# KhutornoyYaroslav/vcm-ts

Measured on AMD Instinct MI355X. Metric: encoded frames/sec at 1920x1080 GOP-32, higher is better.
Workload: dtype f32 (fp16x3 split-MFMA, fp32 accumulate)

## Files before the change

include/dcvc_hip.h:

```cpp
#ifndef DCVC_HIP_H
#define DCVC_HIP_H

#include <stdint.h>

#ifdef __cplusplus
extern "C" {
#endif

#define DCVC_OK 0
#define DCVC_E_ARG (-1)
#define DCVC_E_LAUNCH (-2)
#define DCVC_E_RANGE (-3)

#define DCVC_STATUS_ACT_SATURATED 1

#define DCVC_MAX_SEG 3

#define DCVC_PREC_FP32 0
#define DCVC_PREC_FP16X3 1

typedef struct {
    const float *ptr;
    int32_t C;
    int32_t cs;
} dcvc_seg;

typedef struct {
    dcvc_seg seg[DCVC_MAX_SEG];
    int32_t nseg;
    int32_t N, Hin, Win;
    int32_t in_act;
    float in_slope;
    const float *wpack;
    const float *bpack;
    int32_t ks;
    int32_t stride;
    int32_t Cout;
    int32_t Cout_pad;
    float *out;
    int32_t out_cs;
    int32_t out_act;
    float out_slope;
    int32_t pixel_shuffle;
    const float *res;
    int32_t res_cs;
    const float *res_gate;
    const float *res2;
    int32_t res2_cs;
    int32_t precision;
    int32_t *status;
    float *chan_partial;
    int32_t tile_row0;
    int32_t tile_rows;
    int32_t pair_taps;
} dcvc_conv_args;

int32_t dcvc_conv_tile_rows(int32_t ks, int32_t stride);

int32_t dcvc_conv_chan_partial_parts(int32_t ks, int32_t stride, int32_t Hout, int32_t Wout);
int dcvc_channel_mean_finish(const float *chan_partial, int32_t parts, int32_t row_stride, float *mean, int32_t N,
                             int32_t C, int32_t HW, void *stream);

int64_t dcvc_conv_pack_size(int32_t Cout, int32_t ks, int32_t nseg, const int32_t *seg_C, int32_t *cout_pad);

int dcvc_conv_pack_weights(const float *w, const float *b, int32_t Cout, int32_t ks, int32_t nseg,
                           const int32_t *seg_C, int32_t pixel_shuffle, int32_t precision, float *wpack,
                           float *bpack);

int64_t dcvc_conv_pack_size_paired(int32_t Cout, int32_t Cin, int32_t *cout_pad);
int dcvc_conv_pack_weights_paired(const float *w, const float *b, int32_t Cout, int32_t Cin, float *wpack, float *bpack);

int dcvc_conv2d(const dcvc_conv_args *a, void *stream);
int dcvc_conv_set_lookahead(int32_t mode);

int64_t dcvc_conv_small_pack_bytes(int32_t Cout, int32_t ks, int32_t nseg, const int32_t *seg_C);
int dcvc_conv_small_pack_weights(const float *w, const float *b, int32_t Cout, int32_t ks, int32_t nseg,
                                 const int32_t *seg_C, void *wpack, float *bpack);
int dcvc_conv2d_small(const dcvc_conv_args *a, void *stream);

int64_t dcvc_conv_k32_pack_bytes(int32_t Cout, int32_t ks, int32_t nseg, const int32_t *seg_C, int32_t *cout_pad);
int dcvc_conv_k32_pack_weights(const float *w, const float *b, int32_t Cout, int32_t ks, int32_t nseg,
                               const int32_t *seg_C, int32_t pixel_shuffle, void *wpack, float *bpack);
int dcvc_conv2d_k32(const dcvc_conv_args *a, void *stream);
int dcvc_conv_k32_set_waves(int32_t waves);

int dcvc_warp(const float *src, int32_t src_cs, const float *flow, int32_t flow_cs, float *out, int32_t out_cs,
              int32_t N, int32_t H, int32_t W, int32_t C, void *stream);
int dcvc_up2(const float *src, int32_t src_cs, float *out, int32_t out_cs, float *out2, int32_t out2_cs,
             int32_t N, int32_t H, int32_t W, int32_t C, float scale, void *stream);
int dcvc_down2(const float *src, int32_t src_cs, float *out, int32_t out_cs, int32_t N, int32_t H, int32_t W,
               int32_t C, float scale, int32_t avgpool_order, void *stream);
int dcvc_maxpool2(const float *src, int32_t src_cs, float *out, int32_t out_cs, int32_t N, int32_t H, int32_t W,
                  int32_t C, void *stream);
int dcvc_copy_channels(const float *src, int32_t src_cs, float *out, int32_t out_cs, int64_t npix, int32_t C,
                       void *stream);
int dcvc_nchw_to_nhwc(const float *src, float *out, int32_t out_cs, int32_t N, int32_t C, int32_t H, int32_t W,
                      void *stream);
int dcvc_nhwc_to_nchw(const float *src, int32_t src_cs, float *out, int32_t N, int32_t C, int32_t H, int32_t W,
                      int32_t clamp01, void *stream);

int dcvc_channel_mean(const float *src, int32_t src_cs, float *mean, float *scratch, int32_t N, int32_t HW,
                      int32_t C, void *stream);
int dcvc_se_gate(const float *mean, const float *w1, const float *w2, float *gate, int32_t N, int32_t C,
                 int32_t Cr, void *stream);

int dcvc_scale_channels(const float *src, int32_t src_cs, float *out, int32_t out_cs, const float *q_basic,
                        const float *q_scale, int32_t mode, int32_t N, int32_t HW, int32_t C, void *stream);
int dcvc_scale_channels_map(const float *src, int32_t src_cs, float *out, int32_t out_cs, const float *q_basic,
                            const float *q_scale, int32_t mode, int32_t N, int32_t HW, int32_t C, const float *q_map,
                            int32_t H, int32_t W, void *stream);
int dcvc_round_symbols(const float *z, int32_t z_cs, float *z_hat, int32_t zh_cs, int32_t *sym, int32_t N,
                       int32_t H, int32_t W, int32_t C, void *stream);
int dcvc_symbols_to_nhwc(const int32_t *sym, float *out, int32_t out_cs, int32_t N, int32_t H, int32_t W,
                         int32_t C, void *stream);

typedef struct {
    const float *y;
    int32_t y_cs;
    const float *fusion;
    int32_t fusion_cs;
    const float *spatial;
    int32_t spatial_cs;
    float *params;
    int32_t params_cs;
    float *y_hat;
    float *y_q;
    float *y_res;
    float *scales_hat;
    int32_t *sym;
    int32_t *idx;
    float *out;
    int32_t out_cs;
    const float *q_basic;
    const float *q_scale;
    int32_t N, H, W, C;
    int32_t step;
    const float *idx_edges;
    const float *forced_q;
    const float *q_map;
} dcvc_dual_prior_args;

int dcvc_scale_indexes(const float *scales, int32_t *idx, int64_t n, const float *idx_edges, void *stream);

int dcvc_dual_prior_enc(const dcvc_dual_prior_args *a, void *stream);
int dcvc_dual_prior_dec_index(const dcvc_dual_prior_args *a, void *stream);
int dcvc_dual_prior_dec_apply(const dcvc_dual_prior_args *a, void *stream);

int dcvc_scale_bits(const float *y_q, const float *scales_hat, float *out, float *scratch, int32_t kind, int32_t N,
                    int64_t per_sample, void *stream);
int dcvc_factorized_bits(const float *z_hat, int32_t z_cs, const float *params, float *out, float *scratch, int32_t N,
                         int32_t HW, int32_t C, void *stream);
int dcvc_sq_err(const float *a, int32_t a_cs, const float *b, int32_t b_cs, float *out, float *scratch, int32_t N,
                int32_t HW, int32_t C, void *stream);

int32_t dcvc_cdf_table_cols(void);
int dcvc_build_scale_cdfs(const float *scales, int32_t n_scales, int32_t kind, int32_t *cdf, int32_t *sizes,
                          int32_t *offsets, void *stream);
int dcvc_build_factorized_cdfs(const float *params, int32_t C, int32_t *cdf, int32_t *sizes, int32_t *offsets, void *stream);

const char *dcvc_hip_version(void);

#ifdef __cplusplus
}
#endif
#endif
```

vcm_ts_amd/csrc/conv_small.hip:

```cpp
#include <hip/hip_runtime.h>
#include <stdint.h>
#include <string.h>

#include "dcvc_hip.h"
#include "kernel_common.h"

namespace {

constexpr int KC = 16;

struct SmallK {
    const float *seg_ptr[DCVC_MAX_SEG];
    int seg_C[DCVC_MAX_SEG];
    int seg_cs[DCVC_MAX_SEG];
    int nseg;
    int H, W;
    int in_act;
    float in_slope;
    const char *wpack;
    const float *bpack;
    int Cout;
    float *out;
    int out_cs, out_act;
    float out_slope;
    const float *res;
    int res_cs;
    int *status;
};

template <int KS>
__global__ __launch_bounds__(256, 3) void conv_small(const SmallK a) {
    constexpr int RPW = 2, BH = 4 * RPW, BW = 32, PAD = KS / 2, PH = BH + KS - 1, PW = BW + KS - 1, T = KS * KS;
    constexpr int TPS = KS, NST = KS;
    constexpr int PATCH_F = PH * PW * 16;
    constexpr int SLAB_F = TPS * 4 * 16 * 4;
    __shared__ __attribute__((aligned(16))) float lds[PATCH_F + SLAB_F];
    char *patch = (char *)lds;
    float *wl = lds + PATCH_F;

    const int tid = threadIdx.x, lane = tid & 63, wave = tid >> 6;
    const int x0 = blockIdx.x * BW, y0 = blockIdx.y * BH, img = blockIdx.z;
    const int pr = lane & 15, g = lane >> 4;

    f32x4 acc[RPW][2];
#pragma unroll
    for (int m = 0; m < RPW; ++m)
#pragma unroll
        for (int hf = 0; hf < 2; ++hf) acc[m][hf] = (f32x4){0.f, 0.f, 0.f, 0.f};

    constexpr int NP = (PH * PW * 4 + 255) / 256, NW = (SLAB_F / 4 + 255) / 256;
    f32x4 rp[NP], rw[NW];
    struct Cursor {
        int s, c0, cg, st;
    };
    auto advance = [&](Cursor &k) {
        if (++k.st == NST) {
            k.st = 0;
            ++k.cg;
            k.c0 += KC;
            if (k.c0 >= a.seg_C[k.s]) {
                ++k.s;
                k.c0 = 0;
            }
        }
    };
    int poff[NP];
    unsigned inpic = 0;
#pragma unroll
    for (int u = 0; u < NP; ++u) {
        const int i = tid + u * 256;
        const int p = i >> 2;
        const int py = p / PW, px = p - py * PW;
        const int gy = y0 - PAD + py, gx = x0 - PAD + px;
        const bool ok = i < PH * PW * 4 && gy >= 0 && gy < a.H && gx >= 0 && gx < a.W;
        poff[u] = ok ? gy * a.W + gx : 0;
        inpic |= (ok ? 1u : 0u) << u;
    }
    auto load_patch = [&](const Cursor &k) {
        const int C = a.seg_C[k.s], cs = a.seg_cs[k.s];
        const float *sp = a.seg_ptr[k.s] + (size_t)img * a.H * a.W * cs;
        const int c = k.c0 + (tid & 3) * 4;
        const int cc = c < C ? c : 0;
#pragma unroll
        for (int u = 0; u < NP; ++u) rp[u] = *(const f32x4 *)(sp + (size_t)poff[u] * cs + cc);
    };
    auto store_patch = [&](const Cursor &k) {
        const int C = a.seg_C[k.s];
#pragma unroll
        for (int u = 0; u < NP; ++u) {
            const int i = tid + u * 256;
            if (i < PH * PW * 4) {
                const int qd = i & 3, p = i >> 2;
                const int c = k.c0 + qd * 4;
                f32x4 v = ((inpic >> u) & 1u) && c < C ? rp[u] : (f32x4){0.f, 0.f, 0.f, 0.f};
                if (c + 3 >= C) {
                    if (c + 1 >= C) v[1] = 0.f;
                    if (c + 2 >= C) v[2] = 0.f;
                    v[3] = 0.f;
                }
                if (a.in_act) {
#pragma unroll
                    for (int e = 0; e < 4; ++e) v[e] = act(v[e], a.in_slope);
                }
                f32x4 sv = v * ACT_SCALE;
#pragma unroll
                for (int e = 0; e < 4; ++e) sv[e] = __builtin_amdgcn_fmed3f(sv[e], -F16_MAX, F16_MAX);
                const f16x4 hi = __builtin_convertvector(sv, f16x4);
                const f16x4 lo = __builtin_convertvector(sv - __builtin_convertvector(hi, f32x4), f16x4);
                const int sw = (p >> 1) & 3, h = qd >> 1;
                char *rec = patch + p * 64 + (qd & 1) * 8;
                *(f16x4 *)(rec + ((h ^ sw) << 4)) = hi;
                *(f16x4 *)(rec + (((2 + h) ^ sw) << 4)) = lo;
            }
        }
    };
    auto load_w = [&](const Cursor &k) {
        const f32x4 *wsrc = (const f32x4 *)(a.wpack + ((size_t)(k.cg * T + k.st * TPS)) * 1024);
#pragma unroll
        for (int u = 0; u < NW; ++u) {
            const int i = tid + u * 256;
            if (i < SLAB_F / 4) rw[u] = wsrc[i];
        }
    };
    auto store_w = [&]() {
#pragma unroll
        for (int u = 0; u < NW; ++u) {
            const int i = tid + u * 256;
            if (i < SLAB_F / 4) *(f32x4 *)&wl[i * 4] = rw[u];
        }
    };

    Cursor cur = {0, 0, 0, 0};
    load_patch(cur);
    load_w(cur);
    const f16x8 zero8 = {0, 0, 0, 0, 0, 0, 0, 0};
    while (cur.s < a.nseg) {
        __syncthreads();
        if (cur.st == 0) store_patch(cur);
        store_w();
        __syncthreads();
        Cursor nxt = cur;
        advance(nxt);
        if (nxt.s < a.nseg) {
            if (nxt.st == 0) load_patch(nxt);
            load_w(nxt);
        }
#pragma unroll
        for (int tt = 0; tt < TPS; ++tt) {
            const f16x8 b1 = *(const f16x8 *)&wl[((tt * 4 + (g & 1)) * 16 + pr) * 4];
            const f16x8 b2 = g < 2 ? *(const f16x8 *)&wl[((tt * 4 + 2 + g) * 16 + pr) * 4] : zero8;
#pragma unroll
            for (int m = 0; m < RPW; ++m)
#pragma unroll
                for (int hf = 0; hf < 2; ++hf) {
                    const int p = (wave * RPW + m + cur.st) * PW + hf * 16 + pr + tt;
                    const f16x8 av = *(const f16x8 *)(patch + p * 64 + ((g ^ ((p >> 1) & 3)) << 4));
                    acc[m][hf] = __builtin_amdgcn_mfma_f32_16x16x32_f16(av, b1, acc[m][hf], 0, 0, 0);
                    acc[m][hf] = __builtin_amdgcn_mfma_f32_16x16x32_f16(av, b2, acc[m][hf], 0, 0, 0);
                }
        }
        cur = nxt;
    }

    const float inv_scale = 1.f / (ACT_SCALE * WGT_SCALE);
    const int ch = pr;
    bool sat = false;
    if (ch < a.Cout) {
        const float bias = a.bpack[ch];
#pragma unroll
        for (int m = 0; m < RPW; ++m) {
            const int oy = y0 + wave * RPW + m;
            if (oy >= a.H) continue;
            float rv[2][4];
#pragma unroll
            for (int hf = 0; hf < 2; ++hf)
#pragma unroll
                for (int j = 0; j < 4; ++j) {
                    const int ox = x0 + hf * 16 + g * 4 + j;
                    rv[hf][j] = (a.res && ox < a.W) ? a.res[((size_t)(img * a.H + oy) * a.W + ox) * a.res_cs + ch] : 0.f;
                }
#pragma unroll
            for (int hf = 0; hf < 2; ++hf)
#pragma unroll
                for (int j = 0; j < 4; ++j) {
                    const int ox = x0 + hf * 16 + g * 4 + j;
                    if (ox >= a.W) continue;
                    float v = acc[m][hf][j] * inv_scale + bias;
                    if (a.out_act == 1) v = act(v, a.out_slope);
                    else if (a.out_act == 2) v = fminf(fmaxf(v, 0.f), 1.f);
                    if (a.res) v += rv[hf][j];
                    if (a.status && !(fabsf(v) <= ACT_LIMIT)) sat = true;
                    a.out[((size_t)(img * a.H + oy) * a.W + ox) * a.out_cs + ch] = v;
                }
        }
    }
    if (sat) atomicOr(a.status, DCVC_STATUS_ACT_SATURATED);
}

}

extern "C" int64_t dcvc_conv_small_pack_bytes(int32_t Cout, int32_t ks, int32_t nseg, const int32_t *seg_C) {
    if (Cout <= 0 || Cout > 16 || nseg <= 0 || nseg > DCVC_MAX_SEG || (ks != 3 && ks != 7)) return DCVC_E_ARG;
    int chunks = 0;
    for (int s = 0; s < nseg; ++s) {
        if (seg_C[s] <= 0) return DCVC_E_ARG;
        chunks += (seg_C[s] + KC - 1) / KC;
    }
    return (int64_t)chunks * ks * ks * 1024;
}

extern "C" int dcvc_conv_small_pack_weights(const float *w, const float *b, int32_t Cout, int32_t ks, int32_t nseg,
                                            const int32_t *seg_C, void *wpack, float *bpack) {
    const int64_t total = dcvc_conv_small_pack_bytes(Cout, ks, nseg, seg_C);
    if (total < 0 || !w || !wpack || !bpack) return DCVC_E_ARG;
    const int T = ks * ks;
    int Cin = 0;
    for (int s = 0; s < nseg; ++s) Cin += seg_C[s];
    memset(wpack, 0, (size_t)total);
    for (int n = 0; n < 16; ++n) bpack[n] = (b && n < Cout) ? b[n] : 0.f;
    _Float16 *base = (_Float16 *)wpack;
    int status = DCVC_OK, cg = 0, cin0 = 0;
    for (int s = 0; s < nseg; ++s) {
        for (int c0 = 0; c0 < seg_C[s]; c0 += KC, ++cg)
            for (int t = 0; t < T; ++t)
                for (int cc = 0; cc < KC && c0 + cc < seg_C[s]; ++cc)
                    for (int n = 0; n < Cout; ++n) {
                        float sv = w[((size_t)n * Cin + cin0 + c0 + cc) * T + t] * WGT_SCALE;
                        if (!(fabsf(sv) <= F16_MAX)) { status = DCVC_E_RANGE; sv = sv > 0.f ? F16_MAX : -F16_MAX; }
                        const SplitF16 p = split_f16(sv);
                        const size_t blk = ((size_t)cg * T + t) * 4;
                        base[((blk + (cc >> 3)) * 16 + n) * 8 + (cc & 7)] = p.hi;
                        base[((blk + 2 + (cc >> 3)) * 16 + n) * 8 + (cc & 7)] = p.lo;
                    }
        cin0 += seg_C[s];
    }
    return status;
}

extern "C" int dcvc_conv2d_small(const dcvc_conv_args *a, void *stream) {
    if (!conv_args_ok(a)) return DCVC_E_ARG;
    if (a->out_act < 0 || a->out_act > 2) return DCVC_E_ARG;
    if (a->tile_rows > 0) return DCVC_E_ARG;
    if (a->Cout <= 0 || a->Cout > 16 || (a->ks != 3 && a->ks != 7) || a->stride != 1 || a->pixel_shuffle || a->res_gate ||
        a->res2 || a->chan_partial || a->precision != DCVC_PREC_FP16X3 || a->N <= 0)
        return DCVC_E_ARG;
    SmallK k;
    memset(&k, 0, sizeof(k));
    copy_conv_args(k, a);
    k.H = a->Hin, k.W = a->Win;
    dim3 grid((unsigned)((a->Win + 31) / 32), (unsigned)((a->Hin + 7) / 8), (unsigned)a->N);
    if (a->ks == 7)
        hipLaunchKernelGGL(conv_small<7>, grid, dim3(256), 0, (hipStream_t)stream, k);
    else
        hipLaunchKernelGGL(conv_small<3>, grid, dim3(256), 0, (hipStream_t)stream, k);
    RET_LAUNCH();
}
```

vcm_ts_amd/lib.py:

```python
from __future__ import annotations

import ctypes as C
import functools
import os

HERE = os.path.dirname(os.path.abspath(__file__))
CSRC = os.path.join(HERE, "csrc")


class LibraryMissing(RuntimeError):
    pass


class KernelError(RuntimeError):
    pass


def _load(name):
    path = os.environ.get("DCVC_HIP_LIB") if name == "libdcvc_hip.so" and os.environ.get("DCVC_HIP_LIB") else \
        os.path.join(CSRC, name)
    if not os.path.exists(path):
        raise LibraryMissing(f"{path} not built; run `make -C {CSRC}` (no CPU fallback exists)")
    return C.CDLL(path)


@functools.lru_cache(maxsize=None)
def rans():
    L = _load("libdcvc_rans.so")
    L.dcvc_rans_encoder_create.restype = C.c_void_p
    L.dcvc_rans_encoder_destroy.argtypes = [C.c_void_p]
    L.dcvc_rans_encoder_reset.argtypes = [C.c_void_p]
    L.dcvc_rans_encoder_encode_with_indexes.argtypes = [C.c_void_p, C.c_void_p, C.c_void_p, C.c_int64, C.c_void_p,
                                                        C.c_int32, C.c_int32, C.c_void_p, C.c_void_p]
    L.dcvc_rans_encoder_flush_bound.argtypes = [C.c_void_p]
    L.dcvc_rans_encoder_flush_bound.restype = C.c_int64
    L.dcvc_rans_encoder_flush.argtypes = [C.c_void_p, C.c_void_p, C.c_int64]
    L.dcvc_rans_encoder_flush.restype = C.c_int64
    L.dcvc_rans_decoder_create.restype = C.c_void_p
    L.dcvc_rans_decoder_destroy.argtypes = [C.c_void_p]
    L.dcvc_rans_decoder_set_stream.argtypes = [C.c_void_p, C.c_char_p, C.c_int64]
    L.dcvc_rans_decoder_decode_stream.argtypes = [C.c_void_p, C.c_void_p, C.c_int64, C.c_void_p, C.c_int32,
                                                  C.c_int32, C.c_void_p, C.c_void_p, C.c_void_p]
    L.dcvc_pmf_to_quantized_cdf.argtypes = [C.c_void_p, C.c_int32, C.c_int32, C.c_void_p]
    return L


class Seg(C.Structure):
    _fields_ = [("ptr", C.c_void_p), ("C", C.c_int32), ("cs", C.c_int32)]


class ConvArgs(C.Structure):
    _fields_ = [
        ("seg", Seg * 3), ("nseg", C.c_int32), ("N", C.c_int32), ("Hin", C.c_int32), ("Win", C.c_int32),
        ("in_act", C.c_int32), ("in_slope", C.c_float), ("wpack", C.c_void_p), ("bpack", C.c_void_p),
        ("ks", C.c_int32), ("stride", C.c_int32), ("Cout", C.c_int32), ("Cout_pad", C.c_int32),
        ("out", C.c_void_p), ("out_cs", C.c_int32), ("out_act", C.c_int32), ("out_slope", C.c_float),
        ("pixel_shuffle", C.c_int32), ("res", C.c_void_p), ("res_cs", C.c_int32), ("res_gate", C.c_void_p),
        ("res2", C.c_void_p), ("res2_cs", C.c_int32), ("precision", C.c_int32), ("status", C.c_void_p),
        ("chan_partial", C.c_void_p), ("tile_row0", C.c_int32), ("tile_rows", C.c_int32), ("pair_taps", C.c_int32),
    ]


class DualPriorArgs(C.Structure):
    _fields_ = [
        ("y", C.c_void_p), ("y_cs", C.c_int32), ("fusion", C.c_void_p), ("fusion_cs", C.c_int32),
        ("spatial", C.c_void_p), ("spatial_cs", C.c_int32), ("params", C.c_void_p), ("params_cs", C.c_int32),
        ("y_hat", C.c_void_p), ("y_q", C.c_void_p), ("y_res", C.c_void_p), ("scales_hat", C.c_void_p),
        ("sym", C.c_void_p), ("idx", C.c_void_p), ("out", C.c_void_p), ("out_cs", C.c_int32),
        ("q_basic", C.c_void_p), ("q_scale", C.c_void_p), ("N", C.c_int32), ("H", C.c_int32), ("W", C.c_int32),
        ("C", C.c_int32), ("step", C.c_int32), ("idx_edges", C.c_void_p), ("forced_q", C.c_void_p),
        ("q_map", C.c_void_p),
    ]


class ConvBwdArgs(C.Structure):
    _fields_ = [
        ("dout", C.c_void_p), ("dout_cs", C.c_int32), ("out", C.c_void_p), ("out_cs", C.c_int32),
        ("res", C.c_void_p), ("res_cs", C.c_int32), ("gate", C.c_void_p), ("res2", C.c_void_p), ("res2_cs", C.c_int32),
        ("dres", C.c_void_p), ("dres_cs", C.c_int32), ("dres2", C.c_void_p), ("dres2_cs", C.c_int32),
        ("dpre", C.c_void_p), ("dpre_cs", C.c_int32), ("zs", C.c_int32), ("Hd", C.c_int32), ("Wd", C.c_int32),
        ("N", C.c_int32), ("Ho", C.c_int32), ("Wo", C.c_int32), ("Cout", C.c_int32), ("pixel_shuffle", C.c_int32),
        ("act", C.c_int32), ("slope", C.c_float),
    ]


class WgradArgs(C.Structure):
    _fields_ = [
        ("x", C.c_void_p), ("x_cs", C.c_int32), ("C", C.c_int32), ("in_act", C.c_int32), ("in_slope", C.c_float),
        ("dpre", C.c_void_p), ("dpre_cs", C.c_int32), ("zs", C.c_int32), ("Hd", C.c_int32), ("Wd", C.c_int32),
        ("N", C.c_int32), ("Hin", C.c_int32), ("Win", C.c_int32), ("Ho", C.c_int32), ("Wo", C.c_int32),
        ("Cout", C.c_int32), ("ks", C.c_int32), ("stride", C.c_int32), ("dw", C.c_void_p), ("Cin_total", C.c_int32),
        ("cin_offset", C.c_int32), ("scratch", C.c_void_p), ("scratch_floats", C.c_int64), ("overwrite", C.c_int32),
        ("db", C.c_void_p), ("precision", C.c_int32),
    ]


class PackJob(C.Structure):
    _fields_ = [
        ("w", C.c_void_p), ("b", C.c_void_p), ("Cout", C.c_int32), ("Cin_total", C.c_int32), ("ks", C.c_int32),
        ("nseg", C.c_int32), ("seg_C", C.c_int32 * 3), ("cin_offset", C.c_int32), ("pixel_shuffle", C.c_int32),
        ("precision", C.c_int32), ("transposed", C.c_int32), ("wpack", C.c_void_p), ("bpack", C.c_void_p),
    ]


class DualPriorBwdArgs(C.Structure):
    _fields_ = [
        ("y", C.c_void_p), ("y_cs", C.c_int32), ("fusion", C.c_void_p), ("fusion_cs", C.c_int32),
        ("y_hat", C.c_void_p), ("dout", C.c_void_p), ("dout_cs", C.c_int32), ("dy_res", C.c_void_p),
        ("dscales_hat", C.c_void_p), ("dparams", C.c_void_p), ("dparams_cs", C.c_int32),
        ("dspatial", C.c_void_p), ("dspatial_cs", C.c_int32), ("dy", C.c_void_p), ("dy_cs", C.c_int32),
        ("dfusion", C.c_void_p), ("dfusion_cs", C.c_int32), ("dq_plane", C.c_void_p),
        ("q_basic", C.c_void_p), ("q_scale", C.c_void_p), ("N", C.c_int32), ("H", C.c_int32), ("W", C.c_int32),
        ("C", C.c_int32), ("step", C.c_int32),
    ]


class ColorCoeffs(C.Structure):
    _fields_ = [(n, C.c_float) for n in ("y_off", "c_off", "y_scale", "c_scale", "crr", "cgb", "cgr", "cbb", "kr", "kg", "kb",
                                         "icb", "icr", "y_range", "c_range")] + \
               [(n, C.c_int32) for n in ("max_code", "bit_depth", "siting", "matrix", "range")]


class RoiBox(C.Structure):
    _fields_ = [(n, C.c_int32) for n in ("x1", "y1", "x2", "y2", "cls")]


class RoiClassRec(C.Structure):
    _fields_ = [("border", C.c_int32), ("shrink", C.c_int32), ("feather", C.c_float * 64)]


PRECISIONS = {"fp32": 0, "fp16x3": 1}

i32, i64, f32, vp = C.c_int32, C.c_int64, C.c_float, C.c_void_p

HEADERS = {
    "dcvc_hip.h": {
        "dcvc_conv_tile_rows": (i32, i32, i32),
        "dcvc_conv_chan_partial_parts": (i32, i32, i32, i32, i32),
        "dcvc_channel_mean_finish": [vp, i32, i32, vp, i32, i32, i32, vp],
        "dcvc_conv_pack_size": (i64, i32, i32, i32, vp, C.POINTER(i32)),
        "dcvc_conv_pack_weights": [vp, vp, i32, i32, i32, vp, i32, i32, vp, vp],
        "dcvc_conv_pack_size_paired": (i64, i32, i32, C.POINTER(i32)),
        "dcvc_conv_pack_weights_paired": [vp, vp, i32, i32, vp, vp],
        "dcvc_conv2d": [C.POINTER(ConvArgs), vp],
        "dcvc_conv_set_lookahead": [i32],
        "dcvc_conv_small_pack_bytes": (i64, i32, i32, i32, vp),
        "dcvc_conv_small_pack_weights": [vp, vp, i32, i32, i32, vp, vp, vp],
        "dcvc_conv2d_small": [C.POINTER(ConvArgs), vp],
        "dcvc_conv_k32_pack_bytes": (i64, i32, i32, i32, vp, C.POINTER(i32)),
        "dcvc_conv_k32_pack_weights": [vp, vp, i32, i32, i32, vp, i32, vp, vp],
        "dcvc_conv2d_k32": [C.POINTER(ConvArgs), vp],
        "dcvc_conv_k32_set_waves": [i32],
        "dcvc_warp": [vp, i32, vp, i32, vp, i32, i32, i32, i32, i32, vp],
        "dcvc_up2": [vp, i32, vp, i32, vp, i32, i32, i32, i32, i32, f32, vp],
        "dcvc_down2": [vp, i32, vp, i32, i32, i32, i32, i32, f32, i32, vp],
        "dcvc_maxpool2": [vp, i32, vp, i32, i32, i32, i32, i32, vp],
        "dcvc_copy_channels": [vp, i32, vp, i32, i64, i32, vp],
        "dcvc_nchw_to_nhwc": [vp, vp, i32, i32, i32, i32, i32, vp],
        "dcvc_nhwc_to_nchw": [vp, i32, vp, i32, i32, i32, i32, i32, vp],
        "dcvc_channel_mean": [vp, i32, vp, vp, i32, i32, i32, vp],
        "dcvc_se_gate": [vp, vp, vp, vp, i32, i32, i32, vp],
        "dcvc_scale_channels": [vp, i32, vp, i32, vp, vp, i32, i32, i32, i32, vp],
        "dcvc_scale_channels_map": [vp, i32, vp, i32, vp, vp, i32, i32, i32, i32, vp, i32, i32, vp],
        "dcvc_round_symbols": [vp, i32, vp, i32, vp, i32, i32, i32, i32, vp],
        "dcvc_symbols_to_nhwc": [vp, vp, i32, i32, i32, i32, i32, vp],
        "dcvc_scale_indexes": [vp, vp, i64, vp, vp],
        "dcvc_dual_prior_enc": [C.POINTER(DualPriorArgs), vp],
        "dcvc_dual_prior_dec_index": [C.POINTER(DualPriorArgs), vp],
        "dcvc_dual_prior_dec_apply": [C.POINTER(DualPriorArgs), vp],
        "dcvc_scale_bits": [vp, vp, vp, vp, i32, i32, i64, vp],
        "dcvc_factorized_bits": [vp, i32, vp, vp, vp, i32, i32, i32, vp],
        "dcvc_sq_err": [vp, i32, vp, i32, vp, vp, i32, i32, i32, vp],
        "dcvc_cdf_table_cols": (i32,),
        "dcvc_build_scale_cdfs": [vp, i32, i32, vp, vp, vp, vp],
        "dcvc_build_factorized_cdfs": [vp, i32, vp, vp, vp, vp],
        "dcvc_hip_version": (C.c_char_p,),
    },
    "dcvc_hip_grad.h": {
        "dcvc_conv_pack_weights_dev": [vp, vp, i32, i32, i32, i32, vp, i32, i32, i32, i32, vp, vp, vp],
        "dcvc_pack_plan_create": [C.POINTER(PackJob), i32, C.POINTER(C.c_void_p)],
        "dcvc_pack_plan_run": [vp, vp],
        "dcvc_pack_plan_destroy": (None, vp),
        "dcvc_conv_bwd_prologue": [C.POINTER(ConvBwdArgs), vp],
        "dcvc_conv_wgrad_scratch_min": (i64, i32, i32, i32),
        "dcvc_conv_wgrad": [C.POINTER(WgradArgs), vp],
        "dcvc_channel_dot": [vp, i32, vp, i32, vp, vp, i32, i32, i32, i32, i32, vp],
        "dcvc_mask_accumulate": [vp, i32, vp, i32, f32, vp, i32, i64, i32, vp],
        "dcvc_add_planes": [vp, i32, vp, i32, vp, i32, i64, i32, vp],
        "dcvc_warp_bwd": [vp, i32, vp, i32, vp, i32, vp, i32, vp, i32, i32, i32, i32, i32, vp, vp],
        "dcvc_up2_bwd": [vp, i32, vp, i32, i32, i32, i32, i32, f32, vp],
        "dcvc_down2_bwd": [vp, i32, vp, i32, i32, i32, i32, i32, f32, vp],
        "dcvc_maxpool2_bwd": [vp, i32, vp, i32, vp, i32, i32, i32, i32, i32, vp],
        "dcvc_se_bwd": [vp, vp, vp, vp, vp, vp, vp, vp, i32, i32, i32, vp],
        "dcvc_add_channel_vec": [vp, i32, vp, f32, i32, i32, i32, vp],
        "dcvc_scale_channels_bwd": [vp, i32, vp, i32, vp, vp, i32, i32, i32, i32, vp],
        "dcvc_q_finish": [vp, vp, vp, vp, vp, vp, i32, i32, vp],
        "dcvc_dual_prior_bwd": [C.POINTER(DualPriorBwdArgs), vp],
        "dcvc_scale_bits_bwd": [vp, vp, vp, vp, vp, i32, i32, i64, vp],
        "dcvc_factorized_bits_bwd": [vp, i32, vp, vp, vp, i32, vp, i32, i32, i32, vp],
        "dcvc_sq_err_bwd": [vp, i32, vp, i32, vp, vp, i32, i32, i32, i32, vp],
    },
    "dcvc_hip_rans.h": {
        "dcvc_drans_default_lanes": (i32, i64),
        "dcvc_drans_scratch_words": (i64, i64, i32),
        "dcvc_drans_build_lut": [vp, i32, i32, vp, vp],
        "dcvc_drans_encode": [vp, vp, i32, i32, i64, vp, i32, i32, vp, vp, i32, vp, i64, vp, i64, vp, vp, vp, vp],
        "dcvc_drans_decode": [vp, i64, vp, vp, vp, i32, i32, i64, vp, i32, i32, vp, vp, vp, i32, vp, vp, vp],
    },
    "dcvc_hip_metrics.h": {
        "dcvc_ms_ssim": [vp, vp, i32, i32, i32, i32, i32, i64, i32, i64, f32, i32, vp, vp, vp, vp, vp],
        "dcvc_ms_ssim_grad": [vp, vp, i32, i32, i32, i32, i32, i64, i32, i64, f32, i32, vp, vp, vp, vp],
        "dcvc_ms_ssim_workspace_bytes": (i64, i32, i32, i32, i32, i32),
    },
    "dcvc_hip_color.h": {
        "dcvc_color_coeffs": [i32, i32, i32, i32, vp],
        "dcvc_yuv420_to_rgb": [vp, vp, vp, i32, i32, i32, i32, vp, vp, i32, i32, i32, i64, i32, vp],
        "dcvc_rgb_to_yuv420": [vp, i32, i32, i32, i64, vp, vp, vp, vp, i32, i32, vp, vp, vp, i32, i32, vp, vp],
    },
    "dcvc_hip_roi.h": {
        "dcvc_roi_residual": [vp, i32, i64, vp, i32, i64, i32, i32, vp, vp, i32, vp, i64, i64, i32, i32, i32, i32, vp],
        "dcvc_roi_fuse": [vp, i32, i64, vp, i64, i64, i32, i32, i32, i32, i32, i32, vp, vp, i32, vp, i32, vp, i32, i64, vp],
        "dcvc_roi_sse": [vp, i32, i64, vp, i32, i64, i32, i32, vp, vp, i32, vp, i32, vp, vp],
        "dcvc_roi_qmap": [i32, i32, vp, vp, i32, i32, vp, i32, vp, vp],
    },
    "dcvc_hip_roil.h": {
        "dcvc_roil_cells": [i32, i32, vp, i32, vp, vp, i32],
        "dcvc_roil_check": [vp, i64, vp, i32],
        "dcvc_roil_encode": [vp, i32, i64, vp, i32, i64, i32, i32, vp, vp, i32, i32, vp, i32, vp, vp, i64, vp, vp],
        "dcvc_roil_decode": [vp, vp, i64, i32, i32, vp, vp, i32, vp, vp, i64, i64, i32, i32, i32, i32, vp, vp],
    },
    "dcvc_hip_scene.h": {"dcvc_scene_hist": [vp, i32, i64, i32, i32, vp, vp]},
    "dcvc_hip_bits.h": {
        "dcvc_bits_map_scale": [vp, vp, vp, vp, vp, i32, i32, vp, vp, vp, i32, i32, i32, i32, vp, vp],
        "dcvc_bits_map_factorized": [vp, vp, i32, i32, vp, vp, vp, i32, i32, i32, i32, vp, vp],
        "dcvc_bits_regions": [vp, vp, i32, vp, i32, i32, i32, vp, vp],
        "dcvc_bits_sweep_scale": [vp, vp, vp, vp, i32, vp, i32, i32, vp, vp, vp, i32, i32, i32, i32, vp, vp],
    },
    "dcvc_hip_hash.h": {
        "dcvc_hash_pixels": [vp, i32, i64, i32, i32, vp, vp, vp],
        "dcvc_hash_f32": [vp, i32, i64, i32, i32, i32, vp, vp, vp],
    },
    "dcvc_hip_scale.h": {"dcvc_scale_planes": [vp, i32, i64, vp, i32, i64, i32, i32, i32, i32, i32, vp, vp, vp, vp, i32, vp, vp, vp, vp, i32, vp]},
    "dcvc_hip_aq.h": {
        "dcvc_aq_activity": [vp, i32, i64, i32, i32, vp, vp, vp],
        "dcvc_aq_map": [vp, vp, i32, i32, vp, vp, vp, vp, vp],
    },
    "dcvc_hip_motion.h": {"dcvc_motion_step": [vp, i32, i64, i32, i32, vp, i32, i32, i32, i32, vp, vp]},
    "dcvc_hip_tnr.h": {"dcvc_tnr_step": [vp, i32, i64, vp, i32, i64, vp, i32, i64, i32, i32, vp, i32, vp, vp, vp]},
    "dcvc_hip_redact.h": {"dcvc_redact": [vp, i32, i64, vp, i32, i64, i32, i32, vp, vp, i32, i32, i32, i32, i32, vp, vp]},
}


def _signature(entry):
    return (entry[0], list(entry[1:])) if isinstance(entry, tuple) else (C.c_int, entry)


ALL_HIP_SYMBOLS = [name for funcs in HEADERS.values() for name in funcs]
_SIGS = {name: _signature(e)[1] for funcs in HEADERS.values() for name, e in funcs.items() if isinstance(e, list) or e[0] is None}
_CORE = ("dcvc_hip.h", "dcvc_hip_grad.h", "dcvc_hip_rans.h")
HIP_SYMBOLS = sorted(name for h in _CORE for name in HEADERS[h])
(METRICS_SYMBOLS, COLOR_SYMBOLS, ROI_SYMBOLS, ROIL_SYMBOLS, SCENE_SYMBOLS, BITS_SYMBOLS, HASH_SYMBOLS, SCALE_SYMBOLS, AQ_SYMBOLS,
 MOTION_SYMBOLS, TNR_SYMBOLS, REDACT_SYMBOLS) = (list(funcs) for h, funcs in HEADERS.items() if h not in _CORE)
HASH_CONSTANTS = ["dcvc_hash_chunk_bytes", "dcvc_hash_block_bytes", "dcvc_hash_scratch_bytes"]
RANS_SYMBOLS = [
    "dcvc_rans_encoder_create", "dcvc_rans_encoder_destroy", "dcvc_rans_encoder_reset",
    "dcvc_rans_encoder_encode_with_indexes", "dcvc_rans_encoder_flush_bound", "dcvc_rans_encoder_flush",
    "dcvc_rans_decoder_create", "dcvc_rans_decoder_destroy", "dcvc_rans_decoder_set_stream",
    "dcvc_rans_decoder_decode_stream", "dcvc_pmf_to_quantized_cdf",
]


@functools.lru_cache(maxsize=None)
def hip():
    L = _load("libdcvc_hip.so")
    for funcs in HEADERS.values():
        for name, entry in funcs.items():
            fn = getattr(L, name)
            fn.restype, fn.argtypes = _signature(entry)
    return L


def hash_constant(name):
    return int(i32.in_dll(hip(), name).value)


def check(code, what):
    if code != 0:
        raise KernelError(f"{what} failed with status {code}")
```

Baseline: 42.30.

## Double-buffer weight slabs and software-pipeline fragment reads in small-Cout conv

Adds a lookahead schedule (on by default) for the small-Cout fp16x3 conv kernel. Weight slabs are now double-buffered in LDS, and fragment reads for the next tap are issued before the current tap's MFMAs. Each channel chunk's stages are unrolled, which drops one barrier per stage and precomputes swizzled patch addresses. For ks=7 it also removes bounds branches by having excess threads restage a duplicate slot. The cost is more LDS and more registers per block, which may reduce occupancy at launch_bounds(256,3).

```diff
diff --git a/include/dcvc_hip.h b/include/dcvc_hip.h
--- a/include/dcvc_hip.h
+++ b/include/dcvc_hip.h
@@ -77,6 +77,7 @@
 int dcvc_conv_small_pack_weights(const float *w, const float *b, int32_t Cout, int32_t ks, int32_t nseg,
                                  const int32_t *seg_C, void *wpack, float *bpack);
 int dcvc_conv2d_small(const dcvc_conv_args *a, void *stream);
+int dcvc_conv_small_set_schedule(int32_t mode);
 
 int64_t dcvc_conv_k32_pack_bytes(int32_t Cout, int32_t ks, int32_t nseg, const int32_t *seg_C, int32_t *cout_pad);
 int dcvc_conv_k32_pack_weights(const float *w, const float *b, int32_t Cout, int32_t ks, int32_t nseg,
diff --git a/vcm_ts_amd/csrc/conv_small.hip b/vcm_ts_amd/csrc/conv_small.hip
--- a/vcm_ts_amd/csrc/conv_small.hip
+++ b/vcm_ts_amd/csrc/conv_small.hip
@@ -1,6 +1,7 @@
 #include <hip/hip_runtime.h>
 #include <stdint.h>
 #include <string.h>
+#include <type_traits>
 
 #include "dcvc_hip.h"
 #include "kernel_common.h"
@@ -28,13 +29,17 @@
     int *status;
 };
 
-template <int KS>
+int g_small_schedule = 2;
+
+template <int KS, bool AHEAD>
 __global__ __launch_bounds__(256, 3) void conv_small(const SmallK a) {
     constexpr int RPW = 2, BH = 4 * RPW, BW = 32, PAD = KS / 2, PH = BH + KS - 1, PW = BW + KS - 1, T = KS * KS;
     constexpr int TPS = KS, NST = KS;
     constexpr int PATCH_F = PH * PW * 16;
     constexpr int SLAB_F = TPS * 4 * 16 * 4;
-    __shared__ __attribute__((aligned(16))) float lds[PATCH_F + SLAB_F];
+    constexpr int NSLAB = AHEAD ? 2 : 1;
+    constexpr bool BFREE = AHEAD && KS == 7;
+    __shared__ __attribute__((aligned(16))) float lds[PATCH_F + NSLAB * SLAB_F];
     char *patch = (char *)lds;
     float *wl = lds + PATCH_F;
 
@@ -48,31 +53,44 @@
 #pragma unroll
         for (int hf = 0; hf < 2; ++hf) acc[m][hf] = (f32x4){0.f, 0.f, 0.f, 0.f};
 
-    constexpr int NP = (PH * PW * 4 + 255) / 256, NW = (SLAB_F / 4 + 255) / 256;
+    constexpr int NSLOT = PH * PW * 4, NROW = SLAB_F / 4;
+    constexpr int NP = (NSLOT + 255) / 256, NW = (NROW + 255) / 256;
+    static_assert(!BFREE || (NSLOT > 256 && NROW > 256), "a thread past the end restages its previous slot");
     f32x4 rp[NP], rw[NW];
     struct Cursor {
         int s, c0, cg, st;
     };
+    auto next_chunk = [&](Cursor &k) {
+        ++k.cg;
+        k.c0 += KC;
+        if (k.c0 >= a.seg_C[k.s]) {
+            ++k.s;
+            k.c0 = 0;
+        }
+    };
     auto advance = [&](Cursor &k) {
         if (++k.st == NST) {
             k.st = 0;
-            ++k.cg;
-            k.c0 += KC;
-            if (k.c0 >= a.seg_C[k.s]) {
-                ++k.s;
-                k.c0 = 0;
-            }
-        }
+            next_chunk(k);
+        }
+    };
+    auto pslot = [&](int u) {
+        const int i = tid + u * 256;
+        return BFREE && i >= NSLOT ? i - 256 : i;
+    };
+    auto wslot = [&](int u) {
+        const int i = tid + u * 256;
+        return BFREE && i >= NROW ? i - 256 : i;
     };
     int poff[NP];
     unsigned inpic = 0;
 #pragma unroll
     for (int u = 0; u < NP; ++u) {
-        const int i = tid + u * 256;
+        const int i = pslot(u);
         const int p = i >> 2;
         const int py = p / PW, px = p - py * PW;
         const int gy = y0 - PAD + py, gx = x0 - PAD + px;
-        const bool ok = i < PH * PW * 4 && gy >= 0 && gy < a.H && gx >= 0 && gx < a.W;
+        const bool ok = i < NSLOT && gy >= 0 && gy < a.H && gx >= 0 && gx < a.W;
         poff[u] = ok ? gy * a.W + gx : 0;
         inpic |= (ok ? 1u : 0u) << u;
     }
@@ -84,23 +102,31 @@
 #pragma unroll
         for (int u = 0; u < NP; ++u) rp[u] = *(const f32x4 *)(sp + (size_t)poff[u] * cs + cc);
     };
+    const float slope = a.in_act ? a.in_slope : 1.f;
     auto store_patch = [&](const Cursor &k) {
         const int C = a.seg_C[k.s];
 #pragma unroll
         for (int u = 0; u < NP; ++u) {
-            const int i = tid + u * 256;
-            if (i < PH * PW * 4) {
+            const int i = pslot(u);
+            if (BFREE || i < NSLOT) {
                 const int qd = i & 3, p = i >> 2;
                 const int c = k.c0 + qd * 4;
-                f32x4 v = ((inpic >> u) & 1u) && c < C ? rp[u] : (f32x4){0.f, 0.f, 0.f, 0.f};
-                if (c + 3 >= C) {
-                    if (c + 1 >= C) v[1] = 0.f;
-                    if (c + 2 >= C) v[2] = 0.f;
-                    v[3] = 0.f;
-                }
-                if (a.in_act) {
-#pragma unroll
-                    for (int e = 0; e < 4; ++e) v[e] = act(v[e], a.in_slope);
+                f32x4 v;
+                if (BFREE) {
+                    const int nc = ((inpic >> u) & 1u) ? C - c : 0;
+#pragma unroll
+                    for (int e = 0; e < 4; ++e) v[e] = act(e < nc ? rp[u][e] : 0.f, slope);
+                } else {
+                    v = ((inpic >> u) & 1u) && c < C ? rp[u] : (f32x4){0.f, 0.f, 0.f, 0.f};
+                    if (c + 3 >= C) {
+                        if (c + 1 >= C) v[1] = 0.f;
+                        if (c + 2 >= C) v[2] = 0.f;
+                        v[3] = 0.f;
+                    }
+                    if (a.in_act) {
+#pragma unroll
+                        for (int e = 0; e < 4; ++e) v[e] = act(v[e], a.in_slope);
+                    }
                 }
                 f32x4 sv = v * ACT_SCALE;
 #pragma unroll
@@ -114,52 +140,121 @@
             }
         }
     };
-    auto load_w = [&](const Cursor &k) {
-        const f32x4 *wsrc = (const f32x4 *)(a.wpack + ((size_t)(k.cg * T + k.st * TPS)) * 1024);
+    auto load_w = [&](int cg, int st) {
+        const f32x4 *wsrc = (const f32x4 *)(a.wpack + ((size_t)(cg * T + st * TPS)) * 1024);
 #pragma unroll
         for (int u = 0; u < NW; ++u) {
-            const int i = tid + u * 256;
-            if (i < SLAB_F / 4) rw[u] = wsrc[i];
-        }
-    };
-    auto store_w = [&]() {
+            const int i = wslot(u);
+            if (BFREE || i < NROW) rw[u] = wsrc[i];
+        }
+    };
+    auto store_w = [&](float *w) {
 #pragma unroll
         for (int u = 0; u < NW; ++u) {
-            const int i = tid + u * 256;
-            if (i < SLAB_F / 4) *(f32x4 *)&wl[i * 4] = rw[u];
-        }
-    };
-
-    Cursor cur = {0, 0, 0, 0};
-    load_patch(cur);
-    load_w(cur);
+            const int i = wslot(u);
+            if (BFREE || i < NROW) *(f32x4 *)&w[i * 4] = rw[u];
+        }
+    };
+
     const f16x8 zero8 = {0, 0, 0, 0, 0, 0, 0, 0};
-    while (cur.s < a.nseg) {
-        __syncthreads();
-        if (cur.st == 0) store_patch(cur);
-        store_w();
-        __syncthreads();
+    if constexpr (!AHEAD) {
+        Cursor cur = {0, 0, 0, 0};
+        load_patch(cur);
+        load_w(cur.cg, cur.st);
+        while (cur.s < a.nseg) {
+            __syncthreads();
+            if (cur.st == 0) store_patch(cur);
+            store_w(wl);
+            __syncthreads();
+            Cursor nxt = cur;
+            advance(nxt);
+            if (nxt.s < a.nseg) {
+                if (nxt.st == 0) load_patch(nxt);
+                load_w(nxt.cg, nxt.st);
+            }
+#pragma unroll
+            for (int tt = 0; tt < TPS; ++tt) {
+                const f16x8 b1 = *(const f16x8 *)&wl[((tt * 4 + (g & 1)) * 16 + pr) * 4];
+                const f16x8 b2 = g < 2 ? *(const f16x8 *)&wl[((tt * 4 + 2 + g) * 16 + pr) * 4] : zero8;
+#pragma unroll
+                for (int m = 0; m < RPW; ++m)
+#pragma unroll
+                    for (int hf = 0; hf < 2; ++hf) {
+                        const int p = (wave * RPW + m + cur.st) * PW + hf * 16 + pr + tt;
+                        const f16x8 av = *(const f16x8 *)(patch + p * 64 + ((g ^ ((p >> 1) & 3)) << 4));
+                        acc[m][hf] = __builtin_amdgcn_mfma_f32_16x16x32_f16(av, b1, acc[m][hf], 0, 0, 0);
+                        acc[m][hf] = __builtin_amdgcn_mfma_f32_16x16x32_f16(av, b2, acc[m][hf], 0, 0, 0);
+                    }
+            }
+            cur = nxt;
+        }
+    } else {
+        struct Frag {
+            f16x8 b1, b2, av[RPW][2];
+        };
+        const int p0 = wave * RPW * PW + pr;
+        const char *arec[8];
+#pragma unroll
+        for (int r = 0; r < 8; ++r) arec[r] = patch + p0 * 64 + ((g ^ (((p0 + r) >> 1) & 3)) << 4);
+        auto read_frag = [&](const float *w, int st, int tt) {
+            Frag f;
+            f.b1 =*(const f16x8 *)&w[((tt * 4 + (g & 1)) * 16 + pr) * 4];
+            const f16x8 lo = *(const f16x8 *)&w[((tt * 4 + 2 + (g & 1)) * 16 + pr) * 4];
+            f.b2 = g < 2 ? lo : zero8;
+#pragma unroll
+            for (int m = 0; m < RPW; ++m)
+#pragma unroll
+                for (int hf = 0; hf < 2; ++hf) {
+                    const int k = (m + st) * PW + hf * 16 + tt;
+                    f.av[m][hf] = *(const f16x8 *)(arec[k & 7] + k * 64);
+                }
+            return f;
+        };
+        auto chunk = [&](const Cursor &cur, const Cursor &nxt, auto req) {
+            constexpr bool REQ = decltype(req)::value;
+#pragma unroll
+            for (int st = 0; st < NST; ++st) {
+                float *w = wl + (st & 1) * SLAB_F;
+                if (st == 0) {
+                    __syncthreads();
+                    store_patch(cur);
+                }
+                store_w(w);
+                __syncthreads();
+                if (st + 1 < NST) load_w(cur.cg, st + 1);
+                else if (REQ) load_w(nxt.cg, 0);
+                if (st == 0 && REQ) load_patch(nxt);
+                __builtin_amdgcn_sched_barrier(0);
+                Frag f = read_frag(w, st, 0);
+#pragma unroll
+                for (int tt = 0; tt < TPS; ++tt) {
+                    Frag n = f;
+                    if (tt + 1 < TPS) n = read_frag(w, st, tt + 1);
+#pragma unroll
+                    for (int m = 0; m < RPW; ++m)
+#pragma unroll
+                        for (int hf = 0; hf < 2; ++hf)
+                            acc[m][hf] = __builtin_amdgcn_mfma_f32_16x16x32_f16(f.av[m][hf], f.b1, acc[m][hf], 0, 0, 0);
+#pragma unroll
+                    for (int m = 0; m < RPW; ++m)
+#pragma unroll
+                        for (int hf = 0; hf < 2; ++hf)
+                            acc[m][hf] = __builtin_amdgcn_mfma_f32_16x16x32_f16(f.av[m][hf], f.b2, acc[m][hf], 0, 0, 0);
+                    f = n;
+                }
+            }
+        };
+        Cursor cur = {0, 0, 0, 0};
+        load_patch(cur);
+        load_w(0, 0);
         Cursor nxt = cur;
-        advance(nxt);
-        if (nxt.s < a.nseg) {
-            if (nxt.st == 0) load_patch(nxt);
-            load_w(nxt);
-        }
-#pragma unroll
-        for (int tt = 0; tt < TPS; ++tt) {
-            const f16x8 b1 = *(const f16x8 *)&wl[((tt * 4 + (g & 1)) * 16 + pr) * 4];
-            const f16x8 b2 = g < 2 ? *(const f16x8 *)&wl[((tt * 4 + 2 + g) * 16 + pr) * 4] : zero8;
-#pragma unroll
-            for (int m = 0; m < RPW; ++m)
-#pragma unroll
-                for (int hf = 0; hf < 2; ++hf) {
-                    const int p = (wave * RPW + m + cur.st) * PW + hf * 16 + pr + tt;
-                    const f16x8 av = *(const f16x8 *)(patch + p * 64 + ((g ^ ((p >> 1) & 3)) << 4));
-                    acc[m][hf] = __builtin_amdgcn_mfma_f32_16x16x32_f16(av, b1, acc[m][hf], 0, 0, 0);
-                    acc[m][hf] = __builtin_amdgcn_mfma_f32_16x16x32_f16(av, b2, acc[m][hf], 0, 0, 0);
-                }
-        }
-        cur = nxt;
+        next_chunk(nxt);
+        while (nxt.s < a.nseg) {
+            chunk(cur, nxt, std::true_type());
+            cur = nxt;
+            next_chunk(nxt);
+        }
+        chunk(cur, nxt, std::false_type());
     }
 
     const float inv_scale = 1.f / (ACT_SCALE * WGT_SCALE);
@@ -249,9 +344,20 @@
     copy_conv_args(k, a);
     k.H = a->Hin, k.W = a->Win;
     dim3 grid((unsigned)((a->Win + 31) / 32), (unsigned)((a->Hin + 7) / 8), (unsigned)a->N);
-    if (a->ks == 7)
-        hipLaunchKernelGGL(conv_small<7>, grid, dim3(256), 0, (hipStream_t)stream, k);
+    const bool ahead = g_small_schedule == 2;
+    if (a->ks == 7 && ahead)
+        hipLaunchKernelGGL((conv_small<7, true>), grid, dim3(256), 0, (hipStream_t)stream, k);
+    else if (a->ks == 7)
+        hipLaunchKernelGGL((conv_small<7, false>), grid, dim3(256), 0, (hipStream_t)stream, k);
+    else if (ahead)
+        hipLaunchKernelGGL((conv_small<3, true>), grid, dim3(256), 0, (hipStream_t)stream, k);
     else
-        hipLaunchKernelGGL(conv_small<3>, grid, dim3(256), 0, (hipStream_t)stream, k);
+        hipLaunchKernelGGL((conv_small<3, false>), grid, dim3(256), 0, (hipStream_t)stream, k);
     RET_LAUNCH();
 }
+
+extern "C" int dcvc_conv_small_set_schedule(int32_t mode) {
+    if (mode != 1 && mode != 2) return DCVC_E_ARG;
+    g_small_schedule = mode;
+    return DCVC_OK;
+}
diff --git a/vcm_ts_amd/lib.py b/vcm_ts_amd/lib.py
--- a/vcm_ts_amd/lib.py
+++ b/vcm_ts_amd/lib.py
@@ -147,6 +147,7 @@
         "dcvc_conv_small_pack_bytes": (i64, i32, i32, i32, vp),
         "dcvc_conv_small_pack_weights": [vp, vp, i32, i32, i32, vp, vp, vp],
         "dcvc_conv2d_small": [C.POINTER(ConvArgs), vp],
+        "dcvc_conv_small_set_schedule": [i32],
         "dcvc_conv_k32_pack_bytes": (i64, i32, i32, i32, vp, C.POINTER(i32)),
         "dcvc_conv_k32_pack_weights": [vp, vp, i32, i32, i32, vp, i32, vp, vp],
         "dcvc_conv2d_k32": [C.POINTER(ConvArgs), vp],
```

After: 42.55 (median of 6 runs). Within noise of the previous version (+0.6%).
